# yell/boltzmann-machines

Measured on AMD Instinct MI355X. Metric: Gibbs-steps/sec (CD-k, 784x1024 RBM, batch 512), higher is better.
Workload: dtype f32

## Files before the change

### boltzmann_machines_amd/csrc/bm_gemm.h

```cpp
#pragma once
#include <hip/hip_runtime.h>
#include <stdint.h>
#include <stdlib.h>
#include <string.h>

namespace bm {

struct NoSide {
    static constexpr bool kFinalSync = true;
    static constexpr bool kSplitFill = false, kCohQ = false;
    static constexpr bool kCanAbort = false;
    __device__ __forceinline__ void wait_inputs() {}
    __device__ __forceinline__ void post_fill() {}
    __device__ __forceinline__ void fill() {}
    __device__ __forceinline__ void drain() {}
};

#define BM_ABL(bit) ((ABL >> (bit)) & 1)

#ifdef BM_KERNELS_ONLY
#define BM_KERNEL static __global__
#else
#define BM_KERNEL __global__
#endif
typedef float f32x4 __attribute__((ext_vector_type(4)));
typedef float f32x2v __attribute__((ext_vector_type(2)));

constexpr int NT = 256;

enum : int { KM = 0, XM = 1 };

template <int WI_, int WJ_, int MI_, int NJ_, int BK_, int NB_ = 4>
struct Geo {
    static constexpr int WI = WI_, WJ = WJ_, MI = MI_, NJ = NJ_, BK = BK_;
    static constexpr int NBUF = NB_;
    static constexpr int PF = NB_ - 1;
    static constexpr int NW = WI * WJ;
    static constexpr int NT = 64 * NW;
    static constexpr int TI = 16 * MI * WI;
    static constexpr int TJ = 16 * NJ * WJ;
    static constexpr int E = 4 * MI;
    static constexpr int P_BUF = TI * BK;
    static constexpr int Q_BUF = TJ * BK;
    static constexpr int SMEM_FLOATS = NBUF * (P_BUF + Q_BUF);
    static constexpr int NPP = P_BUF * 4 / (1024 * NW);
    static constexpr int NPQ = Q_BUF * 4 / (1024 * NW);
    static constexpr int NVP = TI * BK / (4 * NT);
    static constexpr int NVQ = TJ * BK / (4 * NT);
    static constexpr int SP = (MI == 2) ? 8 : 4;
    static constexpr int SQ = (NJ == 2) ? 8 : 4;
    static_assert(MI == 1 || MI == 2, "MI");
    static_assert(NJ == 1 || NJ == 2, "NJ");
    static_assert(BK == 32 || BK == 64, "BK");
    static_assert(NB_ >= 4 && NB_ <= 8, "ring depth");
    static_assert(NPP >= 1 && NPP * 1024 * NW == P_BUF * 4, "P chunk must split into whole DMA pieces per wave");
    static_assert(NPQ >= 1 && NPQ * 1024 * NW == Q_BUF * 4, "Q chunk must split into whole DMA pieces per wave");
    static_assert(NVP >= 1 && NVP * 4 * NT == TI * BK && NVQ >= 1 && NVQ * 4 * NT == TJ * BK, "register path split");
    static_assert(SMEM_FLOATS * 4 <= 160 * 1024 - 1024, "LDS");
};
using GeoAct = Geo<2, 2, 2, 1, 64>;
using GeoAct8 = Geo<2, 4, 1, 1, 64>;
using GeoActS = Geo<2, 2, 1, 1, 64>;
using GeoActS32 = Geo<2, 2, 1, 1, 32>;
using GeoAct32 = Geo<2, 2, 2, 1, 32>;
using GeoGrad = Geo<2, 2, 2, 2, 64>;
using GeoGrad8 = Geo<2, 4, 2, 1, 64>;
using GeoGrad8h = Geo<2, 4, 2, 1, 32>;
using GeoBf3S = Geo<1, 4, 2, 1, 64>;

struct Operand {
    const float *ptr;
    int ld;
    int nx;
    int vec;
};

static inline Operand make_operand(const float *p, int ld, int nx) {
    Operand o;
    o.ptr = p; o.ld = ld; o.nx = nx;
    o.vec = (((uintptr_t)p & 15u) == 0 && (ld & 3) == 0) ? 1 : 0;
    return o;
}

static inline bool operand_fast(const Operand &o, int layout, int K) {
    if (!o.ptr) return true;
    if (!o.vec) return false;
    return layout == KM ? (o.nx % 4 == 0 && o.nx >= 4) : (K % 4 == 0);
}

template <int BK> __device__ __forceinline__ int fx(int row) { return (BK == 64) ? (row & 15) : ((row >> 1) & 7); }
template <int S> __device__ __forceinline__ int fk(int row) { return S * ((row >> 2) & 1); }

template <int L, int TX, int BK, int S>
__device__ __forceinline__ int img_off(int row, int c4) {
// ... 460 lines not shown
        __builtin_amdgcn_sched_barrier(0);
#pragma unroll
        for (int c = 0; c < 2; ++c)
            if (c < nch && !is_dma(c) && !BM_ABL(0)) {
                load_chunk<QL, G, FAST, SEG2, PL>(gr, kr, nch1, i0, j0, c, tid);
                store_chunk<QL, G, SEG2, PL>(gr, kr, nch1, c, sP + (c % NBUF) * P_BUF, sQ + (c % NBUF) * Q_BUF, tid);
            }
        {
            int n_after = 0;
#pragma unroll
            for (int c = 2; c < PF; ++c) n_after += (c < nch && is_dma(c) && !BM_ABL(0)) ? 1 : 0;
            wait_vm_chunks<NPW, PF - 2>(n_after);
        }
    }
    BM_MSTAMP(1);
    if (!BM_ABL(5)) wg_barrier();
    if constexpr (Side::kCanAbort) {
        side.post_fill();
        if (side.aborted) { BM_WAIT_VM(0); return; }
    }
    read_frags<QL, G, ABL, PL>(fa, sP, sQ, wi, wj, lane);
    BM_MSTAMP(2);
    const int klast = (SEG2 && kr.K2 > 0) ? kr.K2 - (nch - nch1 - 1) * BK : kr.K1 - (nch1 - 1) * BK;
    const int nq_last = (klast + 15) / 16;
    constexpr int NM = (BK / 4) * G::MI * G::NJ;
    constexpr int NRP = (PL == XM) ? BK / 16 : BK / 4;
    constexpr int NRQ = (QL == XM) ? (BK / 16) * G::NJ : BK / 4;
    constexpr int NR = NRP + NRQ;
#define BM_SG(mask, n) __builtin_amdgcn_sched_group_barrier(mask, n, 0);
#ifndef BM_SCHED_VARIANT
#define BM_SCHED_VARIANT 0
#endif
#if BM_SCHED_VARIANT == 0
#define BM_SCHED_STEP                                                                             \
    if (DW == G::NW) { _Pragma("unroll") for (int s_ = 0; s_ < NPW; ++s_) { BM_SG(0x008, 1) BM_SG(0x020, 1) } } \
    _Pragma("unroll") for (int s_ = 0; s_ < NR; ++s_) { BM_SG(0x008, 1) BM_SG(0x100, 1) }         \
    BM_SG(0x008, NM)
#elif BM_SCHED_VARIANT == 1
#define BM_SCHED_STEP                                                                             \
    _Pragma("unroll") for (int s_ = 0; s_ < NR; ++s_) { BM_SG(0x008, 1) BM_SG(0x100, 1) }         \
    _Pragma("unroll") for (int s_ = 0; s_ < NPW; ++s_) { BM_SG(0x008, 1) BM_SG(0x020, 1) }        \
    BM_SG(0x008, NM)
#else
#define BM_SCHED_STEP
#endif
    static_assert(NBUF == 4, "the steps below are written for a 4-slot ring");
    int cc = 0;
    const unsigned lds0 = (unsigned)(uintptr_t)(__attribute__((address_space(3))) void *)smem;
    const unsigned ldsPw = lds0 + (unsigned)w * 1024u, ldsQw = lds0 + (unsigned)(NBUF * P_BUF * 4) + (unsigned)w * 1024u;
    bool in2 = false;
    auto chunk_bases = [&](int c, const char *&pb, const char *&qb) {
        const bool s2 = SEG2 && c >= nch1;
        const Operand &P = s2 ? kr.P2 : kr.P1, &Q = s2 ? kr.Q2 : kr.Q1;
        const int kc = s2 ? c - nch1 : c;
        pb = (const char *)P.ptr + (size_t)kc * ((PL == KM) ? (size_t)BK * P.ld * 4 : (size_t)BK * 4);
        qb = (const char *)Q.ptr + (size_t)kc * ((QL == KM) ? (size_t)BK * Q.ld * 4 : (size_t)BK * 4);
    };
#define BM_DMA_AT(CD, SD)                                                                         \
    {                                                                                             \
        if (SEG2 && !in2 && (CD) >= nch1) { in2 = true; pl1 = pl2; }                              \
        const char *pb_, *qb_;                                                                    \
        chunk_bases((CD), pb_, qb_);                                                              \
        if (dmaw) dma_chunk_s<G, DW, Side::kCohQ, (BM_ABL(9) != 0)>(pl1, pb_, qb_, ldsPw + (unsigned)((SD) * P_BUF * 4), \
                                     ldsQw + (unsigned)((SD) * Q_BUF * 4));                       \
    }
#define BM_STEP_Q(FC, FN, S)                                                                      \
    {                                                                                             \
        BM_DMA_AT(cc + PF, ((S) + PF) % NBUF)                                                     \
        read_frags<QL, G, ABL, PL>(FN, sP + (((S) + 1) % NBUF) * P_BUF, sQ + (((S) + 1) % NBUF) * Q_BUF, wi, wj, lane); \
        mfma_frags<G, ABL>(acc, FC);                                                              \
        BM_SCHED_STEP                                                                             \
        if (!BM_ABL(8)) BM_WAIT_VM((PF - 2) * NPW);                                               \
        if (!BM_ABL(5)) wg_barrier();                                                             \
        ++cc;                                                                                     \
    }
#define BM_STEP_T(FC, FN, S1, S2, S3)       \
    {                                                                                             \
        const int cd = cc + PF, cr = cc + 2;                                                      \
        const bool do_dma = cd < nch && is_dma(cd) && !BM_ABL(0);                                 \
        const bool do_reg = cr < nch && !is_dma(cr) && !BM_ABL(0);                                \
        if (cc == last - 1) side.drain();       \
        if (do_reg) load_chunk<QL, G, FAST, SEG2, PL, Side::kCohQ>(gr, kr, nch1, i0, j0, cr, tid); \
        if (do_dma) BM_DMA_AT(cd, S3)                                                             \
        read_frags<QL, G, ABL, PL>(FN, sP + (S1) * P_BUF, sQ + (S1) * Q_BUF, wi, wj, lane);       \
        mfma_frags<G, ABL>(acc, FC);                                                              \
        _Pragma("unroll") for (int s_ = 0; s_ < NR; ++s_) { BM_SG(0x008, 1) BM_SG(0x100, 1) }     \
        BM_SG(0x008, NM)                                                                          \
        if (do_reg) {                                                                             \
            BM_WAIT_VM(0);                                                                        \
            store_chunk<QL, G, SEG2, PL>(gr, kr, nch1, cr, sP + (S2) * P_BUF, sQ + (S2) * Q_BUF, tid); \
        } else if (cr < nch) {                                                                    \
             \
            int n_after = 0;                                                                      \
            _Pragma("unroll") for (int c_ = 3; c_ <= PF; ++c_) n_after += (cc + c_ < nch && is_dma(cc + c_) && !BM_ABL(0)) ? 1 : 0; \
            wait_vm_chunks<NPW, PF - 2>(n_after);                                                 \
        }                                                                                         \
        if (!BM_ABL(5)) wg_barrier();                                                             \
        ++cc;                                                                                     \
    }
#define BM_STEP_TC(FC, FN, S) BM_STEP_T(FC, FN, ((S) + 1) % NBUF, ((S) + 2) % NBUF, ((S) + 3) % NBUF)
#define BM_STEP_TR(FC, FN)    BM_STEP_T(FC, FN, (cc + 1) % NBUF, (cc + 2) % NBUF, (cc + 3) % NBUF)
    constexpr int NWR = G::NVP + G::NVQ;
#ifndef BM_REG_SCHED_VARIANT
#define BM_REG_SCHED_VARIANT 0
#endif
#if BM_REG_SCHED_VARIANT == 0
#define BM_REG_SCHED(RELOAD)                                                                      \
        _Pragma("unroll") for (int s_ = 0; s_ < NWR; ++s_) { BM_SG(0x008, 1) BM_SG(0x200, 1) }    \
        if (RELOAD) { _Pragma("unroll") for (int s_ = 0; s_ < NWR; ++s_) { BM_SG(0x008, 1) BM_SG(0x020, 1) } } \
        _Pragma("unroll") for (int s_ = 0; s_ < NR; ++s_) { BM_SG(0x008, 1) BM_SG(0x100, 1) }     \
        BM_SG(0x008, NM)
#elif BM_REG_SCHED_VARIANT == 1
#define BM_REG_SCHED(RELOAD)                                                                      \
        _Pragma("unroll") for (int s_ = 0; s_ < NR; ++s_) { BM_SG(0x008, (NM >= 64 ? 2 : 1)) BM_SG(0x100, 2) } \
        _Pragma("unroll") for (int s_ = 0; s_ < NWR; ++s_) { BM_SG(0x008, (NM >= 32 ? 2 : 1)) BM_SG(0x200, 1) } \
        if (RELOAD) { _Pragma("unroll") for (int s_ = 0; s_ < NWR; ++s_) { BM_SG(0x008, 1) BM_SG(0x020, 1) } } \
        BM_SG(0x008, NM)
#else
#define BM_REG_SCHED(RELOAD)
#endif
#define BM_STEP_REG(FC, FN, G_, RELOAD, S)                                                        \
    {                                                                                             \
        store_chunk_slim<QL, G, PL>(G_, sP + (((S) + 2) % NBUF) * P_BUF, sQ + (((S) + 2) % NBUF) * Q_BUF, tid); \
        if (RELOAD) load_chunk_slim<QL, G, SEG2, PL>(G_, kr, rp1, rp2, nch1, cc + 4);             \
        read_frags<QL, G, ABL, PL>(FN, sP + (((S) + 1) % NBUF) * P_BUF, sQ + (((S) + 1) % NBUF) * Q_BUF, wi, wj, lane); \
        mfma_frags<G, ABL>(acc, FC);                                                              \
        BM_REG_SCHED(RELOAD)                                                                      \
        if (!BM_ABL(5)) wg_barrier();                                                             \
        ++cc;                                                                                     \
    }
    if (n_reg > 0) {
        int left = n_reg;
#pragma unroll 1
        while (left >= 4) {
            BM_STEP_REG(fa, fb, g0, true, 0)
            BM_STEP_REG(fb, fa, g1, true, 1)
            BM_STEP_REG(fa, fb, g0, true, 2)
            BM_STEP_REG(fb, fa, g1, true, 3)
            left -= 4;
        }
        if (left == 2) {
            BM_STEP_REG(fa, fb, g0, true, 0)
            BM_STEP_REG(fb, fa, g1, true, 1)
            BM_STEP_REG(fa, fb, g0, false, 2)
            BM_STEP_REG(fb, fa, g1, false, 3)
        } else {
            BM_STEP_REG(fa, fb, g0, false, 0)
            BM_STEP_REG(fb, fa, g1, false, 1)
        }
    }
    int n_steady = 0;
    if (FAST && STG != STG_REG && !BM_ABL(6) && !BM_ABL(0))
        while (n_steady + PF < nch) {
            bool all = true;
#pragma unroll
            for (int c_ = 2; c_ <= PF; ++c_) all = all && is_dma(n_steady + c_);
            if (!all) break;
            ++n_steady;
        }
#pragma unroll 1
    for (int q = 0; q < n_steady / 4; ++q) {
        BM_STEP_Q(fa, fb, 0)
        BM_STEP_Q(fb, fa, 1)
        BM_STEP_Q(fa, fb, 2)
        BM_STEP_Q(fb, fa, 3)
    }
    constexpr bool CTS = !(G::NW == 8 && G::MI * G::NJ > 1);
    const int last = nch - 1;
    bool odd = false;
    if (CTS) {
        if ((cc & 3) == 2 && cc < last) {
            BM_STEP_TC(fa, fb, 2)
            if (cc < last) { BM_STEP_TC(fb, fa, 3) } else odd = true;
        }
#pragma unroll 1
        while (cc < last && !odd) {
            BM_STEP_TC(fa, fb, 0)
            if (cc >= last) { odd = true; break; }
            BM_STEP_TC(fb, fa, 1)
            if (cc >= last) break;
            BM_STEP_TC(fa, fb, 2)
            if (cc >= last) { odd = true; break; }
            BM_STEP_TC(fb, fa, 3)
        }
    } else {
#pragma unroll 1
        while (cc < last) {
            BM_STEP_TR(fa, fb)
            if (cc >= last) { odd = true; break; }
            BM_STEP_TR(fb, fa)
        }
    }
    if (odd) fa = fb;
    BM_MSTAMP(3);
    if (last < 1) side.drain();
    mfma_frags_head<G, ABL>(acc, fa, nq_last);
    if (!BM_ABL(5) && Side::kFinalSync) wg_barrier();
    BM_MSTAMP(4);
#undef BM_STEP_TC
#undef BM_STEP_TR
#undef BM_STEP_T
#undef BM_STEP_Q
#undef BM_DMA_AT
#undef BM_STEP_REG
#undef BM_REG_SCHED
#undef BM_SCHED_STEP
#undef BM_SG
}

template <int QL, class G>
__device__ __forceinline__ int lane_j(int l15, int n) {
    return (QL == KM && G::NJ == 2) ? 2 * l15 + n : 16 * n + l15;
}

template <class G>
__device__ __forceinline__ void lane_outputs(const f32x4 (&acc)[G::MI][G::NJ], int n, float (&v)[G::E]) {
#pragma unroll
    for (int r = 0; r < 4; ++r)
#pragma unroll
        for (int t = 0; t < G::MI; ++t) v[G::MI * r + t] = acc[t][n][r];
}

struct TileMap {
    int tiles_i, tiles_j, xi, xj, gj;
    int slab;
    unsigned long long rect[8];
    unsigned int spare[8];
};

static inline TileMap make_tile_map(int tiles_i, int tiles_j, double bytes_i, double bytes_j, int force_xi = 0) {
    static int env_xi = -1, env_gj = 0;
    if (env_xi < 0) {
        const char *e = bm::dbg("xcd_map");
        env_xi = 0;
        if (e) { env_xi = atoi(e); const char *c = strchr(e, ':'); env_gj = c ? atoi(c + 1) : 0; }
    }
    if (env_xi > 0) force_xi = env_xi;
    const bool slab = force_xi < 0;
    if (slab) force_xi = 0;
    const double l2_budget = 2.5 * 1024 * 1024;
    TileMap best;
    memset(&best, 0, sizeof(best));
    best.tiles_i = tiles_i; best.tiles_j = tiles_j; best.xi = 8; best.xj = 1; best.gj = tiles_j;
    best.slab = slab ? 1 : 0;
    double best_cost = -1.0;
    for (int xi = 8; xi >= 1; xi >>= 1) {
        const int xj = 8 / xi;
        if (force_xi > 0 && xi != force_xi) continue;
        const double hi = (double)tiles_i / xi, wj = (double)tiles_j / xj;
        int gj = (int)((l2_budget - 4.0 * bytes_i) / (bytes_j > 1.0 ? bytes_j : 1.0));
        if (gj < 1) gj = 1;
        if (gj > (int)(wj + 0.999)) gj = (int)(wj + 0.999);
        if (env_gj > 0) gj = env_gj;
        const double groups = (double)(((int)(wj + 0.999) + gj - 1) / gj);
        const double cost = 8.0 * (hi * bytes_i * groups + wj * bytes_j);
        if (best_cost < 0.0 || cost < best_cost * 0.999) { best_cost = cost; best.xi = xi; best.xj = xj; best.gj = gj; }
    }
    if (best.gj < 1) best.gj = 1;
    const int nb = tiles_i * tiles_j, q = nb / 8, r = nb % 8;
    int spare = 0;
    for (int x = 0; x < 8; ++x) {
        const int a = x % best.xi, c = x / best.xi;
        const int i0 = a * tiles_i / best.xi, hi = (a + 1) * tiles_i / best.xi - i0;
        const int j0 = c * tiles_j / best.xj, wj = (c + 1) * tiles_j / best.xj - j0;
        best.rect[x] = (unsigned long long)(i0 & 0xFFFF) | (unsigned long long)(hi & 0xFFFF) << 16 |
                       (unsigned long long)(j0 & 0xFFFF) << 32 | (unsigned long long)(wj & 0xFFFF) << 48;
        const int cap = q + (x < r ? 1 : 0), sz = hi * wj;
        const int left = sz > cap ? sz - cap : 0;
        best.spare[x] = (unsigned int)(spare & 0xFFFF) | (unsigned int)(left & 0xFFFF) << 16;
        if (cap > sz) spare += cap - sz;
    }
    return best;
}

__host__ __device__ __forceinline__ int small_div(int a, int b) {
    int q = (int)((float)a / (float)b);
    q -= (q * b > a);
    q += ((q + 1) * b <= a);
    return q;
// ... 56 lines not shown
```

### boltzmann_machines_amd/csrc/bm_kernels.h

```cpp
#pragma once
#include <stdio.h>
#include <stdlib.h>
#include <string.h>
#include "bm_gemm.h"
#include "bm_bf3.h"
#include "bm_numerics.h"
#include "bm_rng.h"

namespace bm {

struct MfCtl { unsigned maxdiff; int done; int steps; float resid; };

struct ActArgs {
    Operand P1, Q1; int K1;
    int p_xm;
    Operand P2, Q2; int K2;
    int I, J;
    const float *bias;
    const float *sigma;
    float mult;
    float bmult;
    int kind;
    int sample;
    int lit;
// ... 53 lines not shown
    uint32_t w[4];
    philox_block(key, idx >> 2, w);
    return (int)(w[idx & 3] % (uint32_t)V);
}
#define FE_FLIP_FROM_KEY (reinterpret_cast<const int *>(uintptr_t(1)))
constexpr int BM_MF_SLOTS = 1024;

__device__ __forceinline__ void draw4(const ActArgs &a, const PhiloxKey &key, unsigned long long flat, int ib, int nvalid,
                                      const float *m, float *s, bool aligned) {
    if (aligned) {
        uint32_t wds[4];
        philox_block(key, flat >> 2, wds);
        if (a.kind == 0) {
#pragma unroll
            for (int r = 0; r < 4; ++r) s[r] = (u32_to_uniform(wds[r]) < m[r]) ? 1.f : 0.f;
        } else {
            float n[4];
            box_muller(wds[0], wds[1], n[0], n[1]);
            box_muller(wds[2], wds[3], n[2], n[3]);
#pragma unroll
            for (int r = 0; r < 4; ++r) s[r] = n[r] * a.sigma[ib + r] + m[r];
        }
    } else {
#pragma unroll
        for (int r = 0; r < 4; ++r) {
            if (r >= nvalid) break;
            const unsigned long long idx = flat + r;
            uint32_t wds[4];
            philox_block(key, idx >> 2, wds);
            if (a.kind == 0) {
                s[r] = (u32_to_uniform(wds[idx & 3]) < m[r]) ? 1.f : 0.f;
            } else {
                float n0, n1;
                const int pr = (int)(idx & 3) >> 1;
                box_muller(wds[2 * pr], wds[2 * pr + 1], n0, n1);
                s[r] = ((idx & 1) ? n1 : n0) * a.sigma[ib + r] + m[r];
            }
        }
    }
}

#ifndef BM_NT_STORES
#define BM_NT_STORES 1
#endif
typedef float f32x2 __attribute__((ext_vector_type(2)));
__device__ __forceinline__ void stream_store4(float *p, float x, float y, float z, float w) {
    if (BM_NT_STORES) __builtin_nontemporal_store((f32x4){x, y, z, w}, reinterpret_cast<f32x4 *>(p));
    else *reinterpret_cast<float4 *>(p) = make_float4(x, y, z, w);
}
__device__ __forceinline__ void stream_store2(float *p, float x, float y) {
    if (BM_NT_STORES) __builtin_nontemporal_store((f32x2){x, y}, reinterpret_cast<f32x2 *>(p));
    else *reinterpret_cast<float2 *>(p) = make_float2(x, y);
}

template <bool CACHED = false>
__device__ __forceinline__ void store4(float *dst, size_t o, const float *v, int nvalid, bool v4) {
    if (v4) {
        if (CACHED) *reinterpret_cast<float4 *>(dst + o) = make_float4(v[0], v[1], v[2], v[3]);
        else stream_store4(dst + o, v[0], v[1], v[2], v[3]);
    } else {
#pragma unroll
        for (int r = 0; r < 4; ++r) if (r < nvalid) dst[o + r] = v[r];
    }
}

template <int MI> struct PhiloxFor { typedef PhiloxPair type; };
template <> struct PhiloxFor<1> { typedef PhiloxOne type; };

__device__ __forceinline__ float wave_max_lane63(float v) {
#define BM_DPP_MAX(ctrl, rmask) v = fmaxf(v, __int_as_float(__builtin_amdgcn_update_dpp(__float_as_int(v), __float_as_int(v), ctrl, rmask, 0xf, false)))
    BM_DPP_MAX(0xb1, 0xf);
    BM_DPP_MAX(0x4e, 0xf);
    BM_DPP_MAX(0x124, 0xf);
    BM_DPP_MAX(0x128, 0xf);
    BM_DPP_MAX(0x142, 0xa);
    BM_DPP_MAX(0x143, 0xc);
#undef BM_DPP_MAX
    return v;
}

template <int E, class Rng, bool MF = false, int NTH = 256> struct ActSide {
    static constexpr bool kFinalSync = false;
    static constexpr bool kSplitFill = false, kCohQ = false, kCanAbort = MF;
    static constexpr bool kMF = MF;
    const float *bias, *sigma;
    const float *prev_row;
    int ib0, I, with_rng;
    float bs[E], sg[E], pv[E];
    Rng rng;
    MfCtl *chk_ctl; const float *chk_slots; int chk_n; float chk_tol; const int *skip; float *s_chk; int aborted, nthreads;

    __device__ __forceinline__ void load_inputs() {
        const float *sp = sigma ? sigma : bias;
        const bool has_sigma = sigma != nullptr;
        if (MF && prev_row) {
            if (E == 4 && ib0 + 3 < I && (((uintptr_t)prev_row & 15u) == 0)) {
                const float4 t = *reinterpret_cast<const float4 *>(prev_row);
                pv[0] = t.x; pv[1] = t.y; pv[2] = t.z; pv[E - 1] = t.w;
            } else {
#pragma unroll
                for (int e = 0; e < E; ++e) pv[e] = (ib0 + e < I) ? prev_row[e] : 0.f;
            }
        }
        if (MF && E == 4 && ib0 + 3 < I && (((uintptr_t)(bias + ib0) & 15u) == 0) && (((uintptr_t)(sp + ib0) & 15u) == 0)) {
            const float4 b = *reinterpret_cast<const float4 *>(bias + ib0), v = *reinterpret_cast<const float4 *>(sp + ib0);
            bs[0] = b.x; bs[1] = b.y; bs[2] = b.z; bs[E - 1] = b.w;
            sg[0] = has_sigma ? v.x : 1.0f; sg[1] = has_sigma ? v.y : 1.0f; sg[2] = has_sigma ? v.z : 1.0f; sg[E - 1] = has_sigma ? v.w : 1.0f;
            return;
        }
#pragma unroll
        for (int e = 0; e < E; ++e) {
            const int i = (ib0 + e < I) ? ib0 + e : I - 1;
            bs[e] = bias[i];
            const float sv = sp[i];
            sg[e] = has_sigma ? sv : 1.0f;
        }
    }
    static constexpr int CHK_MAX = 4096;
    float *s_slots;
    static __device__ __forceinline__ void dma4_lane0(const void *src, float *lds_dst) {
        if ((threadIdx.x & 63) == 0) {
            unsigned keep;
            const unsigned lds_addr = (unsigned)(uintptr_t)(__attribute__((address_space(3))) void *)lds_dst;
            asm volatile("s_mov_b32 %0, m0\n\ts_mov_b32 m0, %2\n\ts_nop 0\n\tglobal_load_lds_dword %1, off\n\ts_mov_b32 m0, %0"
                         : "=&s"(keep) : "v"(src), "s"(__builtin_amdgcn_readfirstlane(lds_addr)) : "memory");
        }
    }
    __device__ __forceinline__ void preload() {
        if constexpr (MF) {
            load_inputs();
            aborted = 0;
            const int w = threadIdx.x >> 6, lane = threadIdx.x & 63;
            if (chk_ctl) {
                for (int p = w; p * 256 < chk_n && p * 256 < CHK_MAX; p += nthreads / 64)
                    dma16(reinterpret_cast<const char *>(chk_slots + 256 * p) + 16 * lane, s_slots + 256 * p);
                if (w == 0) dma4_lane0(&chk_ctl->done, s_slots + CHK_MAX);
            } else if (skip) {
                if (w == 0) dma4_lane0(skip, s_slots + CHK_MAX);
            }
        }
    }
    __device__ __forceinline__ void fill() {
        if (!MF) load_inputs();
        if (with_rng) rng.fill();
    }
    __device__ __forceinline__ void post_fill() {
        if constexpr (MF) {
            if (chk_ctl) {
                constexpr int NR = CHK_MAX / (4 * NTH);
                f32x4 v[NR];
#pragma unroll
                for (int q = 0; q < NR; ++q) {
                    const int e = 4 * ((int)threadIdx.x + q * NTH);
                    v[q] = *reinterpret_cast<const f32x4 *>(s_slots + (e < chk_n ? e : 0));
                }
                float m = 0.f;
#pragma unroll
                for (int q = 0; q < NR; ++q) {
                    const bool in = 4 * ((int)threadIdx.x + q * NTH) < chk_n;
                    m = fmaxf(m, in ? fmaxf(fmaxf(v[q][0], v[q][1]), fmaxf(v[q][2], v[q][3])) : 0.f);
                }
                m = wave_max_lane63(m);
                if ((threadIdx.x & 63) == 63) s_chk[threadIdx.x >> 6] = m;
                wg_barrier();
                m = 0.f;
#pragma unroll
// ... 511 lines not shown
                    const float gr = s1[r] / a.u.N;
                    const float d = a.u.lr * (a.u.mom * a.u.dvb[c] + gr);
                    a.u.dvb[c] = d;
                    a.u.vb[c] = a.u.vb[c] + d;
                }
            }
        }
    } else {
        const int c0 = (wv - nv) * 64;
        block_colsum(a.h0m, a.ldh0, a.hm, a.ldh, c0, a.u.H, a.B, true, smem, s1, s2, a.hm_negated != 0);
        if ((lane & 15) == 0) {
#pragma unroll
            for (int r = 0; r < 4; ++r) {
                const int h = c0 + w * 16 + g * 4 + r;
                if (h < a.u.H) {
                    const float sq = s2[r];
                    a.raw_tail[a.u.V + h] = s1[r];
                    a.raw_tail[a.u.V + a.u.H + h] = sq;
                    if (a.raw_only) continue;
                    const float qn = a.u.damping * a.u.q[h] + (1.0f - a.u.damping) * sq;
                    a.u.q[h] = qn;
                    const float pen = a.u.cost * (qn - a.u.target);
                    a.u.pen[h] = pen;
                    float gr = s1[r] / a.u.N;
                    gr = gr - pen;
                    const float d = a.u.lr * (a.u.mom * a.u.dhb[h] + gr);
                    a.u.dhb[h] = d;
                    a.u.hb[h] = a.u.hb[h] + d;
                }
            }
        }
    }
}

BM_KERNEL __launch_bounds__(NT) void rbm_bias_fused_kernel(RbmBiasFusedArgs a) {
    __shared__ __attribute__((aligned(16))) float smem[CS_SMEM_FLOATS];
    rbm_bias_fused_block(a, blockIdx.x, smem);
}

struct GradArgs {
    Operand Ppos, Qpos; int Kpos;
    Operand Pneg, Qneg; int Kneg;
    int I, J;
    int form;
    int fused;
    float *raw;
    float *raw2;
    float *W, *dW;
    float *Wt;
    int ldw, ldwt;
    const float *pen;
    float N, M, l2, lr, mom;
    int nbias;
    RbmBiasFusedArgs bias;
    int fetch_at_fill;
    int map_xi;
#ifdef BM_PROBE
    long long *dbg;
#endif
};

__device__ __forceinline__ void apply_w_update(float g, float pen, float l2, float lr, float mom,
                                               float &w, float &dw) {
    g = __fsub_rn(g, __fmul_rn(l2, w));
    g = __fsub_rn(g, pen);
    const float d = __fmul_rn(lr, __fadd_rn(__fmul_rn(mom, dw), g));
    dw = d;
    w = __fadd_rn(w, d);
}
__device__ __forceinline__ bool grad_pow2(float N) { return ((__float_as_uint(N) & 0x007fffffu) == 0u) && N >= 1.0f; }
__device__ __forceinline__ float grad_norm1(float r, float N, float invN, bool pow2) {
    return pow2 ? __fmul_rn(r, invN) : __fdiv_rn(r, N);
}
__device__ __forceinline__ float grad_norm2(float r, float r2, float N, float M, float invN, float invM, bool pow2) {
    return pow2 ? __fsub_rn(__fmul_rn(r, invN), __fmul_rn(r2, invM)) : __fsub_rn(__fdiv_rn(r, N), __fdiv_rn(r2, M));
}

struct DivBy {
    float n, inv; bool pow2;
    __device__ __forceinline__ explicit DivBy(float N) : n(N), inv(1.0f / N),
        pow2(grad_pow2(N)) {}
};

template <int NJ> struct GradSide {
    static constexpr bool kFinalSync = true;
    static constexpr bool kSplitFill = false, kCohQ = false, kCanAbort = false;
    const float *W, *dW; int ldw, I, J, ib0, jb[NJ]; bool on, vec8;
    float4 w[NJ][2], d[NJ][2];
    bool at_fill;
    __device__ __forceinline__ void fill() { if (at_fill) fetch(); }
    __device__ __forceinline__ void drain() { if (!at_fill) fetch(); }
    __device__ __forceinline__ void fetch() {
        if (!on || ib0 >= I) return;
#pragma unroll
        for (int n = 0; n < NJ; ++n) {
            if (jb[n] >= J) continue;
            const size_t o = (size_t)jb[n] * ldw + ib0;
            if (vec8) {
                w[n][0] = *reinterpret_cast<const float4 *>(W + o);  w[n][1] = *reinterpret_cast<const float4 *>(W + o + 4);
                d[n][0] = *reinterpret_cast<const float4 *>(dW + o); d[n][1] = *reinterpret_cast<const float4 *>(dW + o + 4);
            } else {
                float tw[8], td[8];
#pragma unroll
                for (int e = 0; e < 8; ++e) {
                    const bool ok = ib0 + e < I;
                    tw[e] = ok ? W[o + e] : 0.f;
                    td[e] = ok ? dW[o + e] : 0.f;
                }
                w[n][0] = make_float4(tw[0], tw[1], tw[2], tw[3]); w[n][1] = make_float4(tw[4], tw[5], tw[6], tw[7]);
                d[n][0] = make_float4(td[0], td[1], td[2], td[3]); d[n][1] = make_float4(td[4], td[5], td[6], td[7]);
            }
        }
    }
};

struct GradCen { const float *oj, *gj, *oi, *gi; };
__device__ __forceinline__ const GradCen &grad_cen_of(const GradCen &c) { return c; }
template <class G, bool FAST, int ABL = 0, int STG = STG_DMA, int MINB = 1, class... CENP>
BM_KERNEL __launch_bounds__(G::NT, MINB) void grad_kernel(GradArgs a, TileMap tmap, CENP... cenp) {
    constexpr int CEN = (int)sizeof...(CENP);
    static_assert(CEN <= 1, "grad_kernel: at most one GradCen");
    constexpr int TI = G::TI, NJ = G::NJ;
    static_assert(G::MI == 2 && G::TI == 64 && G::TJ == 64, "grad_kernel: 64 x 64 tiles, 8 consecutive outputs per lane");
    __shared__ __attribute__((aligned(16))) float smem[G::SMEM_FLOATS];
    constexpr bool kBias = G::SMEM_FLOATS >= CS_SMEM_FLOATS;
    static_assert(G::NT >= NT, "bias path");
    const int ntile_blocks = (int)gridDim.x - a.nbias;
    if ((int)blockIdx.x >= ntile_blocks) {
        if constexpr (kBias) {
            if (G::NT > NT && threadIdx.x >= NT) return;
            rbm_bias_fused_block(a.bias, (int)blockIdx.x - ntile_blocks, smem);
        }
        return;
    }
    asm volatile("" :: "s"(a.Ppos.ptr), "s"(a.Qpos.ptr), "s"(a.Ppos.ld), "s"(a.Qpos.ld), "s"(a.Ppos.nx), "s"(a.Qpos.nx),
                       "s"(a.Pneg.ptr), "s"(a.Qneg.ptr), "s"(a.Pneg.ld), "s"(a.Qneg.ld), "s"(a.Kpos), "s"(a.Kneg),
                       "s"(a.I), "s"(a.J), "s"(a.W), "s"(a.dW), "s"(a.ldw), "s"(a.form), "s"(a.fused));
    constexpr int TJ2 = G::TJ;
    int ti, tj;
    if (tmap.slab) {
        block_to_tile((a.J + TJ2 - 1) / TJ2, ti, tj, 0, a.nbias);
    } else {
        TILE_WORDS(tmap, (int)blockIdx.x);
        TILE_OF_BLOCK(tmap, (int)blockIdx.x, ntile_blocks, ti, tj);
    }
    const int i0 = ti * TI, j0 = tj * TJ2;
    const int tid = threadIdx.x, lane = tid & 63, w = tid >> 6;
    const int wi = w % G::WI, wj = w / G::WI;
    const int g = lane >> 4, l15 = lane & 15;
    const int ib0 = i0 + wi * 32 + g * 8;

#ifdef BM_PROBE
#define BM_GSTAMP(n) do { if (a.dbg && threadIdx.x == 0) a.dbg[blockIdx.x * 4 + (n)] = (long long)__builtin_readcyclecounter(); } while (0)
#else
#define BM_GSTAMP(n) do {} while (0)
#endif
    BM_GSTAMP(0);
    f32x4 pos[2][NJ], neg[2][NJ];
#pragma unroll
    for (int t = 0; t < 2; ++t)
#pragma unroll
        for (int n = 0; n < NJ; ++n) pos[t][n] = neg[t][n] = (f32x4){0.f, 0.f, 0.f, 0.f};
    GradSide<NJ> side;
    side.W = a.W; side.dW = a.dW; side.ldw = a.ldw; side.I = a.I; side.J = a.J; side.ib0 = ib0;
#pragma unroll
    for (int n = 0; n < NJ; ++n) side.jb[n] = j0 + wj * (16 * NJ) + lane_j<KM, G>(l15, n);
    side.vec8 = (ib0 + 7 < a.I) && ((a.ldw & 3) == 0);
    side.at_fill = true;
    side.on = a.fused != 0 && a.fetch_at_fill != 0;
    KRange kr;
    kr.P1 = a.Ppos; kr.Q1 = a.Qpos; kr.K1 = a.Kpos;
    if (a.form == 0) {
        kr.P2 = a.Pneg; kr.Q2 = a.Qneg; kr.K2 = a.Kneg;
        mainloop<KM, G, FAST, true, ABL, KM, STG>(pos, kr, i0, j0, smem, side);
    } else {
        kr.P2 = a.Ppos; kr.Q2 = a.Qpos; kr.K2 = 0;
        mainloop<KM, G, FAST, false, 0, KM, STG>(pos, kr, i0, j0, smem, side);
        kr.P1 = a.Pneg; kr.Q1 = a.Qneg; kr.K1 = a.Kneg;
        mainloop<KM, G, FAST, false, 0, KM, STG>(neg, kr, i0, j0, smem, side);
    }

    BM_GSTAMP(1);
    if (ib0 >= a.I) return;
    if (!a.fetch_at_fill) { side.on = a.fused != 0; side.fetch(); }
    const DivBy divN(a.N), divM(a.M);
    float wt[NJ][8];
    bool jok[NJ];
    float coi[CEN ? 8 : 1], cgi[CEN ? 8 : 1];
    if constexpr (CEN != 0) {
#pragma unroll
        for (int e = 0; e < 8; ++e) {
            const bool ok = ib0 + e < a.I;
            coi[e] = ok ? grad_cen_of(cenp...).oi[ib0 + e] : 0.f;
            cgi[e] = ok ? grad_cen_of(cenp...).gi[ib0 + e] : 0.f;
        }
    }
#pragma unroll
    for (int n = 0; n < NJ; ++n) {
        const int j = side.jb[n];
        jok[n] = j < a.J;
        if (!jok[n]) continue;
        float pv[8], nv[8];
        lane_outputs<G>(pos, n, pv);
        lane_outputs<G>(neg, n, nv);
        const size_t o = (size_t)j * a.ldw + ib0;
        if (!a.fused) {
#pragma unroll
            for (int e = 0; e < 8; ++e) {
                if (ib0 + e >= a.I) break;
                a.raw[o + e] = pv[e];
                if (a.form != 0) a.raw2[o + e] = nv[e];
            }
            continue;
        }
        float wv[8] = {side.w[n][0].x, side.w[n][0].y, side.w[n][0].z, side.w[n][0].w, side.w[n][1].x, side.w[n][1].y, side.w[n][1].z, side.w[n][1].w};
        float dv[8] = {side.d[n][0].x, side.d[n][0].y, side.d[n][0].z, side.d[n][0].w, side.d[n][1].x, side.d[n][1].y, side.d[n][1].z, side.d[n][1].w};
        float pe[8];
#pragma unroll
        for (int e = 0; e < 8; ++e) pe[e] = (a.pen && ib0 + e < a.I) ? a.pen[ib0 + e] : 0.f;
        float gr[8];
        if (divN.pow2 && divM.pow2) {
#pragma unroll
            for (int e = 0; e < 8; ++e) gr[e] = (a.form == 0) ? grad_norm1(pv[e], a.N, divN.inv, true)
                                                              : grad_norm2(pv[e], nv[e], a.N, a.M, divN.inv, divM.inv, true);
        } else {
#pragma unroll
            for (int e = 0; e < 8; ++e) gr[e] = (a.form == 0) ? grad_norm1(pv[e], a.N, 0.f, false)
                                                              : grad_norm2(pv[e], nv[e], a.N, a.M, 0.f, 0.f, false);
        }
        if constexpr (CEN != 0) {
            const float oj = grad_cen_of(cenp...).oj[j], gj = grad_cen_of(cenp...).gj[j];
#pragma unroll
            for (int e = 0; e < 8; ++e) gr[e] = __fsub_rn(gr[e], __fadd_rn(__fmul_rn(oj, cgi[e]), __fmul_rn(gj, coi[e])));
        }
#pragma unroll
        for (int e = 0; e < 8; ++e) {
            apply_w_update(gr[e], pe[e], a.l2, a.lr, a.mom, wv[e], dv[e]);
            wt[n][e] = wv[e];
        }
        if (side.vec8) {
            stream_store4(a.W + o, wv[0], wv[1], wv[2], wv[3]);
            stream_store4(a.W + o + 4, wv[4], wv[5], wv[6], wv[7]);
            stream_store4(a.dW + o, dv[0], dv[1], dv[2], dv[3]);
            stream_store4(a.dW + o + 4, dv[4], dv[5], dv[6], dv[7]);
        } else {
#pragma unroll
            for (int e = 0; e < 8; ++e)
                if (ib0 + e < a.I) { a.W[o + e] = wv[e]; a.dW[o + e] = dv[e]; }
        }
    }
    if (a.fused && a.Wt) {
        const int ja = side.jb[0];
        const bool pair = NJ == 2 && jok[0] && jok[NJ - 1] && ((a.ldwt & 1) == 0);
#pragma unroll
        for (int e = 0; e < 8; ++e) {
            if (ib0 + e >= a.I) break;
            float *dst = a.Wt + (size_t)(ib0 + e) * a.ldwt + ja;
            if (pair) {
                stream_store2(dst, wt[0][e], wt[NJ - 1][e]);
            } else {
                if (jok[0]) dst[0] = wt[0][e];
                if (NJ == 2 && jok[NJ - 1]) dst[1] = wt[NJ - 1][e];
            }
        }
    }
    BM_GSTAMP(2);
}
// ... 771 lines not shown
```

### boltzmann_machines_amd/csrc/bm_launch.h

```cpp
#pragma once
#include <array>
#include <map>
#include <mutex>
#include "bm_common.h"

namespace bm {

template <class G> static inline int tile_grid(int I, int J) { return ((I + G::TI - 1) / G::TI) * ((J + G::TJ - 1) / G::TJ); }

static inline int device_cu_count() {
    static const int n = [] {
        hipDeviceProp_t pr;
        int d = 0;
        (void)hipGetDevice(&d);
        return (hipGetDeviceProperties(&pr, d) == hipSuccess && pr.multiProcessorCount > 0) ? pr.multiProcessorCount : 256;
    }();
    return n;
}
static inline int dbg_int(const char *name) { const char *e = dbg(name); return e ? atoi(e) : 0; }

constexpr int XI_MODEL = 0, XI_SLAB = -1;
struct Tuned { int geo = 0; int xi = XI_MODEL; };
constexpr int TUNE_REP = 4, TUNE_ROUNDS = 3;
constexpr float NOT_TIMED = 1e30f;
// ... 283 lines not shown
}
void launch_act_cr_as(int geo, const ActArgs &a, hipStream_t st);
static inline void launch_act_cr(const ActArgs &a, hipStream_t st) {
    if (a.K2 > 0 || a.fe_flip || a.prev || a.maxdiff || a.skip || a.chk_ctl || a.acc_init || a.clamp_mask || a.row_mult || a.b3.K1 > 0 ||
        a.lit || a.kind != 3 || a.mult != 1.0f || a.bmult != 1.0f || a.sample || a.rowacc || a.rowdot_out) {
        fprintf(stderr, "bm355: a class-rows pass is a single-segment logits pass of its own flavour (no such kernel)\n");
        abort();
    }
    static const int geo_env = dbg_int("act_geo");
    const int ov = geo_env ? geo_env : a.geo_hint;
    if (ov) { launch_act_cr_as(ov, a, st); return; }
    ActArgs plain = a;
    plain.cr_part = nullptr; plain.cr_U = nullptr; plain.cr_ldu = plain.cr_C = plain.cr_nslots = 0; plain.ld_part = 0;
    const Tuned T = tuned_act(plain, st);
    if (T.xi != XI_MODEL && !a.map_xi) {
        ActArgs a2 = a;
        a2.map_xi = T.xi;
        launch_act_cr_as(T.geo, a2, st);
        return;
    }
    launch_act_cr_as(T.geo, a, st);
}
static inline void launch_act(const ActArgs &a, hipStream_t st) {
    if (a.cr_part) { launch_act_cr(a, st); return; }
    if (a.row_mult) { launch_act_rt(a, st); return; }
    if (a.clamp_mask) { launch_act_cl(a, st); return; }
    if (a.b3.K1 > 0) { launch_act_bf3(a, st); return; }
    if (a.fe_flip) { launch_act_fe(a, st); return; }
    if (a.prev || a.maxdiff || a.skip || a.chk_ctl || a.acc_init) { launch_act_mf(a, st); return; }
    if (a.lit && a.kind == 0) { launch_act_lit(a, st); return; }
    launch_act_f32(a, st);
    if (a.states16 && a.states)
        hipLaunchKernelGGL(shadow16_kernel, dim3(256), dim3(256), 0, st, (const float *)a.states, a.ldo, a.J, a.I, a.states16, a.ld16);
}

template <class G, int STG, int MINB = 1>
static inline void launch_grad_geo(const GradArgs &g, hipStream_t st) {
    const double kt = (double)g.Kpos + (double)g.Kneg;
    const TileMap tmap = make_tile_map((g.I + G::TI - 1) / G::TI, (g.J + G::TJ - 1) / G::TJ, kt * G::TI * 4.0, kt * G::TJ * 4.0, g.map_xi);
    const bool fast = operand_fast(g.Ppos, KM, g.Kpos) && operand_fast(g.Qpos, KM, g.Kpos) &&
                      operand_fast(g.Pneg, KM, g.Kneg) && operand_fast(g.Qneg, KM, g.Kneg);
    const dim3 grid(tile_grid<G>(g.I, g.J) + g.nbias), blk(G::NT);
    if (fast) hipLaunchKernelGGL((grad_kernel<G, true, 0, STG, MINB>), grid, blk, 0, st, g, tmap);
    else      hipLaunchKernelGGL((grad_kernel<G, false, 0, STG_DMA, MINB>), grid, blk, 0, st, g, tmap);
}
void launch_grad_cen(int geo, const GradArgs &g, const GradCen &cen, hipStream_t st);
static inline void launch_grad_as(int geo, const GradArgs &g, hipStream_t st) {
    if (geo == 9 && g.nbias == 0) launch_grad_geo<GeoGrad8h, STG_DMA, 4>(g, st);
    else if (geo == 9)   launch_grad_geo<GeoGrad8, STG_DMA>(g, st);
    else if (geo == 208) launch_grad_geo<GeoGrad8, STG_DMAH>(g, st);
    else if (geo == 108) launch_grad_geo<GeoGrad8, STG_REG>(g, st);
    else if (geo == 104) launch_grad_geo<GeoGrad, STG_REG>(g, st);
    else if (geo == 8)   launch_grad_geo<GeoGrad8, STG_DMA>(g, st);
    else                 launch_grad_geo<GeoGrad, STG_DMA>(g, st);
}
static inline Tuned tune_grad_shape(const GradArgs &g, hipStream_t st) {
    constexpr int NC = 5;
    static const int cand[NC] = {4, 8, 104, 108, 9};
    Tuned T;
    T.geo = 4;
    const size_t mat = (((size_t)g.J * (size_t)g.ldw) + 3) & ~(size_t)3;
    float *s = tune_scratch(4 * mat);
    if (!s) return T;
    GradArgs t = g;
    t.nbias = 0; t.pen = nullptr; t.Wt = nullptr;
    t.W = s; t.dW = s + mat; t.raw = s + 2 * mat; t.raw2 = s + 3 * mat;
    (void)hipMemsetAsync(s, 0, 4 * mat * sizeof(float), st);
#ifdef BM_PROBE
    t.dbg = nullptr;
#endif
    TuneTimer tm;
    if (!tm.init(st)) return T;
    float us[NC], xi_us[5];
    best_of(tm, TUNE_ROUNDS, TUNE_REP, NC, us, [&](int c) { launch_grad_as(cand[c], t, st); });
    const int b = fastest(us, NC);
    if (b >= 0) T.geo = cand[b];
    T.xi = tune_tile_map(tm, t, xi_us, [&] { launch_grad_as(T.geo, t, st); });
    if (tune_log())
        fprintf(stderr, "bm355 tune: grad I=%d J=%d K=%d+%d form=%d fused=%d -> geometry %d (us, dma: 4w %.1f, 8w %.1f; reg: 4w %.1f, 8w %.1f; 8w bk32 x2: %.1f), "
                        "tile map %d (9 slab, else XCD grid xi; us: slab %.1f, 8x1 %.1f, 4x2 %.1f, 2x4 %.1f, 1x8 %.1f)\n",
                g.I, g.J, g.Kpos, g.Kneg, g.form, g.fused, T.geo, us[0], us[1], us[2], us[3], us[4], T.xi == XI_SLAB ? 9 : T.xi, xi_us[4], xi_us[0], xi_us[1], xi_us[2], xi_us[3]);
    return T;
}
static inline void launch_grad(const GradArgs &g_in, hipStream_t st, const GradCen *cen = nullptr) {
    static const int fetch_env = std::max(0, dbg_int("grad_fetch")), geo_env = dbg_int("grad_geo");
    GradArgs g = g_in;
    g.fetch_at_fill = fetch_env;
    if (geo_env) { if (cen) launch_grad_cen(geo_env, g, *cen, st); else launch_grad_as(geo_env, g, st); return; }
    static TuneMemo<6> memo;
    const Tuned T = memo.get({g.I, g.J, g.Kpos, g.Kneg, g.form | (g.fused << 1), g.ldw}, [&] { return tune_grad_shape(g, st); });
    if (T.xi != XI_MODEL && !g.map_xi) g.map_xi = T.xi;
    if (cen) launch_grad_cen((T.geo == 8 || T.geo == 9 || T.geo == 108 || T.geo == 208) ? 8 : 4, g, *cen, st);
    else launch_grad_as(T.geo, g, st);
}

static inline void launch_fe_hidden(const FeArgs &f, hipStream_t st) {
    const bool fast = operand_fast(f.P, KM, f.K) && operand_fast(f.Q, XM, f.K);
    const dim3 grid(tile_grid<GeoAct>(f.I, f.J)), blk(NT);
    if (fast) hipLaunchKernelGGL((fe_hidden_kernel<true>), grid, blk, 0, st, f);
    else      hipLaunchKernelGGL((fe_hidden_kernel<false>), grid, blk, 0, st, f);
}

static inline void launch_apply_w(const ApplyWArgs &a, const RbmBiasArgs *bias, hipStream_t st) {
    const bool tiled = (a.I % 4 == 0) && (a.ldw % 4 == 0) && (!a.Wt || a.ldwt % 4 == 0);
    if (tiled) {
        RbmBiasArgs b;
        memset(&b, 0, sizeof(b));
        int nb = 0;
        if (bias) { b = *bias; nb = (b.V + b.H + 255) / 256; }
        const int ntile = ((a.I + 63) / 64) * ((a.J + 63) / 64);
        hipLaunchKernelGGL(apply_w_tiled_kernel, dim3(ntile + nb), dim3(256), 0, st, a, b, nb);
    } else {
        if (bias) hipLaunchKernelGGL(rbm_bias_kernel, dim3((bias->V + bias->H + 255) / 256), dim3(256), 0, st, *bias);
        hipLaunchKernelGGL(apply_w_kernel, dim3(1024), dim3(256), 0, st, a);
    }
}
#endif

}
```

Before: 15770.

## Prefetch W and dW tiles into LDS via DMA during grad mainloop tail

Adds a mid-loop hook to the GEMM mainloop. After the last K-chunk's DMA has been issued, it reuses the freed LDS slot to asynchronously copy the weight and momentum tile (W, dW) needed by the fused update epilogue. The epilogue then reads these values from LDS instead of doing global loads after the loop, hiding that latency behind the final MFMA steps. This becomes the default fetch mode (2). It adds one extra VM-counter wait and only applies to full 64x64 aligned tiles, so it risks slightly stalling the last step.

```diff
diff --git a/boltzmann_machines_amd/csrc/bm_gemm.h b/boltzmann_machines_amd/csrc/bm_gemm.h
--- a/boltzmann_machines_amd/csrc/bm_gemm.h
+++ b/boltzmann_machines_amd/csrc/bm_gemm.h
@@ -10,6 +10,7 @@
     static constexpr bool kFinalSync = true;
     static constexpr bool kSplitFill = false, kCohQ = false;
     static constexpr bool kCanAbort = false;
+    static constexpr bool kHasMid = false;
     __device__ __forceinline__ void wait_inputs() {}
     __device__ __forceinline__ void post_fill() {}
     __device__ __forceinline__ void fill() {}
@@ -636,6 +637,14 @@
         if (cc == last - 1) side.drain();       \
         if (do_reg) load_chunk<QL, G, FAST, SEG2, PL, Side::kCohQ>(gr, kr, nch1, i0, j0, cr, tid); \
         if (do_dma) BM_DMA_AT(cd, S3)                                                             \
+        bool do_mid = false;                    \
+        if constexpr (Side::kHasMid) {                                                            \
+            do_mid = mid_ok && cd == nch;                                                         \
+            if (do_mid) {                                                                         \
+                if (dmaw) side.template mid<G, DW>(ldsPw + (unsigned)((S3) * P_BUF * 4), ldsQw + (unsigned)((S3) * Q_BUF * 4), w, lane); \
+                side.mid_slot = (S3);                                                             \
+            }                                                                                     \
+        }                                                                                         \
         read_frags<QL, G, ABL, PL>(FN, sP + (S1) * P_BUF, sQ + (S1) * Q_BUF, wi, wj, lane);       \
         mfma_frags<G, ABL>(acc, FC);                                                              \
         _Pragma("unroll") for (int s_ = 0; s_ < NR; ++s_) { BM_SG(0x008, 1) BM_SG(0x100, 1) }     \
@@ -647,6 +656,7 @@
              \
             int n_after = 0;                                                                      \
             _Pragma("unroll") for (int c_ = 3; c_ <= PF; ++c_) n_after += (cc + c_ < nch && is_dma(cc + c_) && !BM_ABL(0)) ? 1 : 0; \
+            if (do_mid) n_after += 1;                    \
             wait_vm_chunks<NPW, PF - 2>(n_after);                                                 \
         }                                                                                         \
         if (!BM_ABL(5)) wg_barrier();                                                             \
@@ -721,6 +731,12 @@
     }
     constexpr bool CTS = !(G::NW == 8 && G::MI * G::NJ > 1);
     const int last = nch - 1;
+    bool mid_ok = false;
+    if constexpr (Side::kHasMid) {
+        static_assert(Side::kFinalSync, "the mid hook's data is published by the final barrier");
+        mid_ok = FAST && STG != STG_REG && ABL == 0 && side.mid_on;
+        side.mid_slot = -1;
+    }
     bool odd = false;
     if (CTS) {
         if ((cc & 3) == 2 && cc < last) {
@@ -749,6 +765,9 @@
     BM_MSTAMP(3);
     if (last < 1) side.drain();
     mfma_frags_head<G, ABL>(acc, fa, nq_last);
+    if constexpr (Side::kHasMid) {
+        if (side.mid_slot >= 0) BM_WAIT_VM(0);
+    }
     if (!BM_ABL(5) && Side::kFinalSync) wg_barrier();
     BM_MSTAMP(4);
 #undef BM_STEP_TC
diff --git a/boltzmann_machines_amd/csrc/bm_kernels.h b/boltzmann_machines_amd/csrc/bm_kernels.h
--- a/boltzmann_machines_amd/csrc/bm_kernels.h
+++ b/boltzmann_machines_amd/csrc/bm_kernels.h
@@ -159,6 +159,7 @@
 template <int E, class Rng, bool MF = false, int NTH = 256> struct ActSide {
     static constexpr bool kFinalSync = false;
     static constexpr bool kSplitFill = false, kCohQ = false, kCanAbort = MF;
+    static constexpr bool kHasMid = false;
     static constexpr bool kMF = MF;
     const float *bias, *sigma;
     const float *prev_row;
@@ -836,14 +837,41 @@
         pow2(grad_pow2(N)) {}
 };
 
-template <int NJ> struct GradSide {
+template <int NJ, bool MID = true> struct GradSide {
     static constexpr bool kFinalSync = true;
     static constexpr bool kSplitFill = false, kCohQ = false, kCanAbort = false;
+    static constexpr bool kHasMid = MID;
     const float *W, *dW; int ldw, I, J, ib0, jb[NJ]; bool on, vec8;
     float4 w[NJ][2], d[NJ][2];
     bool at_fill;
+    bool mid_on;
+    int mid_slot;
+    int i0, j0;
     __device__ __forceinline__ void fill() { if (at_fill) fetch(); }
-    __device__ __forceinline__ void drain() { if (!at_fill) fetch(); }
+    __device__ __forceinline__ void drain() {}
+    template <class G, int DW>
+    __device__ __forceinline__ void mid(unsigned ldsP, unsigned ldsQ, int wave, int lane) {
+        static_assert(G::P_BUF == 64 * 64 && G::Q_BUF == 64 * 64, "a 64 x 64 tile fills one slot image");
+        constexpr int NP = DmaPlan<G, DW>::NPP;
+        static_assert(NP == DmaPlan<G, DW>::NPQ && NP * DW == 16, "16 pieces of 4 rows per image");
+        const int r = 4 * wave + (lane >> 4);
+        const uint32_t voff = (uint32_t)(r * ldw + 4 * ((lane & 15) ^ (r & 15))) * 4u;
+#pragma unroll
+        for (int n = 0; n < NP; ++n)
+            dma16s(W + (size_t)(j0 + 4 * DW * n) * ldw + i0, voff, ldsP + (unsigned)(n * DW * 1024));
+#pragma unroll
+        for (int n = 0; n < NP; ++n)
+            dma16s(dW + (size_t)(j0 + 4 * DW * n) * ldw + i0, voff, ldsQ + (unsigned)(n * DW * 1024));
+    }
+    __device__ __forceinline__ void staged(const float *sW, const float *sD) {
+#pragma unroll
+        for (int n = 0; n < NJ; ++n) {
+            const int jl = jb[n] - j0, c = (ib0 - i0) >> 2;
+            const int o0 = jl * 64 + 4 * (c ^ (jl & 15)), o1 = jl * 64 + 4 * ((c + 1) ^ (jl & 15));
+            w[n][0] = *reinterpret_cast<const float4 *>(sW + o0); w[n][1] = *reinterpret_cast<const float4 *>(sW + o1);
+            d[n][0] = *reinterpret_cast<const float4 *>(sD + o0); d[n][1] = *reinterpret_cast<const float4 *>(sD + o1);
+        }
+    }
     __device__ __forceinline__ void fetch() {
         if (!on || ib0 >= I) return;
 #pragma unroll
@@ -915,13 +943,20 @@
     for (int t = 0; t < 2; ++t)
 #pragma unroll
         for (int n = 0; n < NJ; ++n) pos[t][n] = neg[t][n] = (f32x4){0.f, 0.f, 0.f, 0.f};
-    GradSide<NJ> side;
+    constexpr bool kMid = FAST && STG != STG_REG && ABL == 0 && G::BK == 64;
+    GradSide<NJ, kMid> side;
     side.W = a.W; side.dW = a.dW; side.ldw = a.ldw; side.I = a.I; side.J = a.J; side.ib0 = ib0;
 #pragma unroll
     for (int n = 0; n < NJ; ++n) side.jb[n] = j0 + wj * (16 * NJ) + lane_j<KM, G>(l15, n);
     side.vec8 = (ib0 + 7 < a.I) && ((a.ldw & 3) == 0);
-    side.at_fill = true;
-    side.on = a.fused != 0 && a.fetch_at_fill != 0;
+    const int fmode = a.fused ? a.fetch_at_fill : 0;
+    side.on = a.fused != 0;
+    side.at_fill = fmode == 1;
+    const bool mid_tile = fmode == 2 && i0 + TI <= a.I && j0 + TJ2 <= a.J && (a.ldw & 3) == 0 &&
+                          (((uintptr_t)a.W | (uintptr_t)a.dW) & 15u) == 0;
+    side.mid_on = mid_tile && a.form == 0;
+    side.mid_slot = -1;
+    side.i0 = i0; side.j0 = j0;
     KRange kr;
     kr.P1 = a.Ppos; kr.Q1 = a.Qpos; kr.K1 = a.Kpos;
     if (a.form == 0) {
@@ -931,12 +966,16 @@
         kr.P2 = a.Ppos; kr.Q2 = a.Qpos; kr.K2 = 0;
         mainloop<KM, G, FAST, false, 0, KM, STG>(pos, kr, i0, j0, smem, side);
         kr.P1 = a.Pneg; kr.Q1 = a.Qneg; kr.K1 = a.Kneg;
+        side.at_fill = false;
+        side.mid_on = mid_tile;
         mainloop<KM, G, FAST, false, 0, KM, STG>(neg, kr, i0, j0, smem, side);
     }
 
     BM_GSTAMP(1);
     if (ib0 >= a.I) return;
-    if (!a.fetch_at_fill) { side.on = a.fused != 0; side.fetch(); }
+    const int wslot = kMid ? side.mid_slot : -1;
+    if (wslot >= 0) side.staged(smem + wslot * G::P_BUF, smem + G::NBUF * G::P_BUF + wslot * G::Q_BUF);
+    else if (fmode != 1) side.fetch();
     const DivBy divN(a.N), divM(a.M);
     float wt[NJ][8];
     bool jok[NJ];
diff --git a/boltzmann_machines_amd/csrc/bm_launch.h b/boltzmann_machines_amd/csrc/bm_launch.h
--- a/boltzmann_machines_amd/csrc/bm_launch.h
+++ b/boltzmann_machines_amd/csrc/bm_launch.h
@@ -389,8 +389,10 @@
                 g.I, g.J, g.Kpos, g.Kneg, g.form, g.fused, T.geo, us[0], us[1], us[2], us[3], us[4], T.xi == XI_SLAB ? 9 : T.xi, xi_us[4], xi_us[0], xi_us[1], xi_us[2], xi_us[3]);
     return T;
 }
+constexpr int GRAD_FETCH_DEFAULT = 2;
 static inline void launch_grad(const GradArgs &g_in, hipStream_t st, const GradCen *cen = nullptr) {
-    static const int fetch_env = std::max(0, dbg_int("grad_fetch")), geo_env = dbg_int("grad_geo");
+    static const int fetch_env = dbg("grad_fetch") ? std::max(0, dbg_int("grad_fetch")) : GRAD_FETCH_DEFAULT;
+    static const int geo_env = dbg_int("grad_geo");
     GradArgs g = g_in;
     g.fetch_at_fill = fetch_env;
     if (geo_env) { if (cen) launch_grad_cen(geo_env, g, *cen, st); else launch_grad_as(geo_env, g, st); return; }
```

New measurement: 15860 (median of 6 runs). No clear change (+0.6%).
